# zhouzypaul/fql

Measured on NVIDIA B200. Metric: fql_update_samples_per_sec, higher is better.
Workload: dtype bf16

## Files before the change

fql_b200/csrc/euler_cluster.cu:

```cuda
#include "step.cuh"
#include "tc_prims.cuh"

using namespace tc;

namespace {

constexpr int TILE_M = 128;
constexpr int KB = 64;
constexpr int A_BLK = TILE_M * 128;
constexpr int SUB = 32;
constexpr int A_SUB = TILE_M * SUB * 2;
constexpr int NSUB = 16;
constexpr int MAX_A = 32;
constexpr int NMMA = 4;
#ifndef FQL_EULER_NISS
#define FQL_EULER_NISS 2
#endif
constexpr int NISS = FQL_EULER_NISS;
static_assert(NISS == 1 || NISS == 2 || NISS == 4, "NISS");
constexpr int NEPI = 4;
constexpr int NTHREADS = 32 * (1 + NMMA + NEPI);
constexpr int EPI0 = 32 * (1 + NMMA);

struct EulerArgs {
// ... 112 lines not shown
    const int N = lastl ? a.A : a.H;
    const int col = lastl ? c : (int)j * NCOL + c;
    sBias[i] = (c < NCOL && col < N && !(l == 0 && a.c0)) ? a.params[(int64_t)s * a.arena + a.off_b[l] + col] : 0.f;
  }
  if (threadIdx.x <= a.n_steps) sT[threadIdx.x] = (float)((double)threadIdx.x / (double)a.n_steps);
  tc_fence_before();
  __syncthreads();
  tc_fence_after();
  cluster_sync_all();
  const uint32_t tmem_base = *tmem_slot;
  if (a.t_start && blockIdx.x == 0 && threadIdx.x == 0) a.t_start[0] = gtime();

  if (warp == 0) {
    const bool el = elect_one();
    {
      if (el) mbar_expect_tx(x_full, nkb_x * A_BLK);
      const int xrow = s * a.x_rows_s + a.x_row0 + tile * TILE_M;
      for (int kb = 0; kb < nkb_x; kb++)
        if (el) tma_load_2d(sX + kb * A_BLK, &mapX, x_full, kb * KB, xrow);
      int n_pub = 0;
      int l = 0;
      for (int it = 0; it < total; it++, l = (l + 1 == NL) ? 0 : l + 1) {
        const bool last = (l == NL - 1);
        const int K = (l == 0) ? a.K0 : a.H;
        const int kblocks = (K + KB - 1) / KB;
        if (it > 0) mbar_wait_u(acc_full, (it - 1) & 1);
        if (el) mbar_expect_tx(full_b, kblocks * B_BLK);
        for (int kb = 0; kb < kblocks; kb++) {
          if (!el) continue;
          if constexpr (MODE == MODE_DGRAD) {
// ... 272 lines not shown
  FQL_REQUIRE(smem <= 232448, "euler_cluster_kernel: shared memory %d > 227 KB", smem);
  auto kern = euler_cluster_kernel<NC, AMAX, MODE>;
  static bool attr_set[FQL_MAX_DEVICES] = {};
  const int dev = fql_current_device();
  if (!attr_set[dev]) {
    FQL_CHECK_CUDA(cudaFuncSetAttribute(kern, cudaFuncAttributeMaxDynamicSharedMemorySize, 232448));
    if (NC > 8) FQL_CHECK_CUDA(cudaFuncSetAttribute(kern, cudaFuncAttributeNonPortableClusterSizeAllowed, 1));
    attr_set[dev] = true;
  }
  cudaLaunchConfig_t cfg;
  memset(&cfg, 0, sizeof(cfg));
  cfg.gridDim = dim3(NC * a.tiles * a.S);
  cfg.blockDim = dim3(NTHREADS);
  cfg.dynamicSmemBytes = smem;
  cfg.stream = st;
  cudaLaunchAttribute attr[1];
  attr[0].id = cudaLaunchAttributeClusterDimension;
  attr[0].val.clusterDim.x = NC;
  attr[0].val.clusterDim.y = 1;
  attr[0].val.clusterDim.z = 1;
  cfg.attrs = attr;
  cfg.numAttrs = 1;
  if (query_only) {
    cfg.stream = nullptr;
    if (cudaOccupancyMaxActiveClusters(max_clusters, kern, &cfg) != cudaSuccess) {
      cudaGetLastError();
      *max_clusters = 0;
    }
    return 0;
  }
  const CUtensorMapSwizzle wsw = (NC == 8 || MODE == MODE_DGRAD) ? CU_TENSOR_MAP_SWIZZLE_128B : CU_TENSOR_MAP_SWIZZLE_64B;
  CUtensorMap mapX, mapW, mapWL;
  HMaps mapsH;
  memset(&mapsH, 0, sizeof(mapsH));
  FQL_TRY(make_map_2d(&mapX, f.X0b, a.K0pad, (uint64_t)a.S * f.Mcap0, 64, TILE_M));
  if (MODE == MODE_DGRAD) {
    FQL_TRY(make_map_2d(&mapW, f.shadow, d->hidden, (uint64_t)a.S * a.w_rows_s, 64, NCOL, wsw));
// ... 130 lines not shown
```

fql_b200/csrc/losses.cu:

```cuda
#include "step.cuh"
#include "dp_comm.cuh"

#include <cuda_bf16.h>

namespace {

__device__ __forceinline__ float clip1(float x) { return fminf(fmaxf(x, -1.0f), 1.0f); }

template <int OP>
__device__ float block_reduce(float v, float* sh) {
  const int lane = threadIdx.x & 31, w = threadIdx.x >> 5, nw = (blockDim.x + 31) >> 5;
  v = OP == 0 ? warp_sum(v) : warp_max(v);
  __syncthreads();
  if (lane == 0) sh[w] = v;
  __syncthreads();
  if (w == 0) {
    float x = lane < nw ? sh[lane] : (OP == 0 ? 0.f : -INFINITY);
    x = OP == 0 ? warp_sum(x) : warp_max(x);
    if (lane == 0) sh[0] = x;
  }
  __syncthreads();
  float r = sh[0];
  return r;
}
// ... 196 lines not shown
__global__ void euler_update_kernel(StepShape sh, WsPtrs w, int step) {
  const int A = sh.A, B = sh.B, KF = sh.F + sh.A + 1;
  const int64_t i = (int64_t)blockIdx.x * blockDim.x + threadIdx.x;
  if (i >= (int64_t)sh.S * B * A) return;
  const int c = (int)(i % A);
  const int64_t row = i / A;
  const int s = (int)(row / B), r = (int)(row % B);
  float* xf = w.XF + ((int64_t)s * 2 * B + B + r) * KF;
  const float v = w.F_out[((int64_t)s * 2 * B + B + r) * A + c];
  const float a = xf[sh.F + c] + v / (float)sh.flow_steps;
  xf[sh.F + c] = a;
  if (c == 0) xf[sh.F + A] = (float)((double)(step + 1) / (double)sh.flow_steps);
  if (step == sh.flow_steps - 1) w.target[i] = clip1(a);
}

__global__ void actor_grad_kernel(StepShape sh, FqlHparams hp, WsPtrs w, float* raw, __nv_bfloat16* dapib) {
  __shared__ float red[32];
  const int s = blockIdx.x;
  const int A = sh.A, B = sh.B, KC = sh.F + sh.A;
  const float* api = w.O_out + ((int64_t)s * 3 * B + B) * A;
  const float scale = hp.alpha * 2.0f / ((float)sh.GB * (float)A);
  float sq = 0.f;
  if (dapib) {
    const int P = 64 - A;
    for (int i = blockIdx.y * blockDim.x + threadIdx.x; i < B * P; i += gridDim.y * blockDim.x)
      dapib[((int64_t)s * B + i / P) * 64 + A + i % P] = __float2bfloat16(0.f);
  }
  for (int i = blockIdx.y * blockDim.x + threadIdx.x; i < B * A; i += gridDim.y * blockDim.x) {
    const int r = i / A, c = i % A;
    const float a = api[i];
    const float d = a - w.target[(int64_t)s * B * A + i];
    sq += d * d;
    const float g0 = w.dX0[(((int64_t)s * 2 + 0) * B + r) * KC + sh.F + c];
    const float g1 = w.dX0[(((int64_t)s * 2 + 1) * B + r) * KC + sh.F + c];
    const float inside = (a >= -1.0f && a <= 1.0f) ? 1.0f : 0.0f;
    const float g = scale * d + (g0 + g1) * inside;
    w.dapi[(int64_t)s * B * A + i] = g;
    if (dapib) dapib[((int64_t)s * B + r) * 64 + c] = __float2bfloat16(g);
  }
  sq = block_reduce<0>(sq, red);
  if (threadIdx.x == 0) atomicAdd(&raw[s * FQL_NUM_RAW + RAW_DISTILL_SQ], sq);
}

__global__ void finalize_info_kernel(StepShape sh, FqlHparams hp, const float* raw, int ranks, const float* gstats, float* info,
                                     int with_grad_stats) {
  const int s = blockIdx.x * blockDim.x + threadIdx.x;
  if (s >= sh.S) return;
  fql_finalize_info_seed(sh, hp, raw, ranks, gstats, info, s, with_grad_stats);
}

__global__ void clip_kernel(const float* in, float* out, int64_t n) {
  const int64_t i = (int64_t)blockIdx.x * blockDim.x + threadIdx.x;
  if (i < n) out[i] = clip1(in[i]);
}

__global__ void concat_kernel(const float* x0, int k0, const float* x1, int k1, float c2, int k2, float* out, int64_t rows) {
// ... 46 lines not shown
  FQL_CHECK_LAUNCH();
  return 0;
}
int launch_bc_post(const StepShape& sh, const WsPtrs& w, float* raw, cudaStream_t st) {
  bc_post_kernel<<<dim3(sh.S, loss_ctas(sh)), 1024, 0, st>>>(sh, w, raw);
  FQL_CHECK_LAUNCH();
  return 0;
}
int launch_euler_update(const StepShape& sh, const WsPtrs& w, int step, cudaStream_t st) {
  const int64_t n = (int64_t)sh.S * sh.B * sh.A;
  euler_update_kernel<<<(unsigned)((n + 255) / 256), 256, 0, st>>>(sh, w, step);
  FQL_CHECK_LAUNCH();
  return 0;
}
int launch_actor_grad(const StepShape& sh, const FqlHparams& hp, const WsPtrs& w, float* raw, cudaStream_t st, void* dapib) {
  actor_grad_kernel<<<dim3(sh.S, loss_ctas(sh)), 1024, 0, st>>>(sh, hp, w, raw, reinterpret_cast<__nv_bfloat16*>(dapib));
  FQL_CHECK_LAUNCH();
  return 0;
}
int launch_finalize_info(const StepShape& sh, const FqlHparams& hp, const float* raw, int ranks, const float* gstats, float* info,
                         int with_grad_stats, cudaStream_t st) {
  finalize_info_kernel<<<(sh.S + 63) / 64, 64, 0, st>>>(sh, hp, raw, ranks, gstats, info, with_grad_stats);
  FQL_CHECK_LAUNCH();
  return 0;
}
int launch_clip(const float* in, float* out, int64_t n, cudaStream_t st) {
  if (n == 0) return 0;
  clip_kernel<<<(unsigned)((n + 255) / 256), 256, 0, st>>>(in, out, n);
  FQL_CHECK_LAUNCH();
  return 0;
}
// ... 15 lines not shown
```

fql_b200/csrc/optim.cu:

```cuda
#include "step.cuh"

#include <cuda_bf16.h>

namespace {

constexpr int ADAM_U = 1;
__global__ void __launch_bounds__(256) adam_polyak_stats_kernel(Layout L, FqlHparams hp, float* __restrict__ params,
                                                                float* __restrict__ mu, float* __restrict__ nu,
                                                                const float* __restrict__ grads,
                                                                const float* __restrict__ bc,
                                                                float* __restrict__ partials, __nv_bfloat16* __restrict__ shadow,
                                                                int64_t shadow_seed, int blk0, int blk1, int nblk) {
  const int s = blockIdx.y;
  const int b0 = blk0 + blockIdx.x * ADAM_U;
  const int64_t base = (int64_t)s * L.arena;
  const NetView& tgt = L.net[FQL_NET_TARGET_CRITIC];
  const NetView& cri = L.net[FQL_NET_CRITIC];
  float4 g[ADAM_U], p[ADAM_U], m[ADAM_U], v[ADAM_U], tp[ADAM_U];
  bool act[ADAM_U], pol[ADAM_U];
#pragma unroll
  for (int u = 0; u < ADAM_U; u++) {
    const int64_t off = (int64_t)(b0 + u) * FQL_LEAF_PAD + threadIdx.x * 4;
    act[u] = (b0 + u < blk1) && !(off >= tgt.begin && off < tgt.end);
    pol[u] = act[u] && off >= cri.begin && off < cri.end;
    if (act[u]) {
      g[u] = *reinterpret_cast<const float4*>(grads + base + off);
      p[u] = *reinterpret_cast<const float4*>(params + base + off);
// ... 14 lines not shown
    float pn[4];
    float mx = -INFINITY, mn = INFINITY, sq = 0.f;
#pragma unroll
    for (int i = 0; i < 4; i++) {
      const float gi = gr[i];
      mx = fmaxf(mx, gi);
      mn = fminf(mn, gi);
      sq += gi * gi;
      mr[i] = hp.beta1 * mr[i] + hp.one_minus_beta1 * gi;
      vr[i] = hp.beta2 * vr[i] + hp.one_minus_beta2 * gi * gi;
      const float mhat = mr[i] / bc1;
      const float vhat = vr[i] / bc2;
      pn[i] = pr[i] + (-hp.lr * (mhat / (sqrtf(vhat) + hp.eps)));
    }
    *reinterpret_cast<float4*>(params + base + off) = make_float4(pn[0], pn[1], pn[2], pn[3]);
    if (shadow) {
      __nv_bfloat162 lo = __floats2bfloat162_rn(pn[0], pn[1]), hi = __floats2bfloat162_rn(pn[2], pn[3]);
      *reinterpret_cast<uint2*>(shadow + (int64_t)s * shadow_seed + off) = make_uint2(*reinterpret_cast<uint32_t*>(&lo), *reinterpret_cast<uint32_t*>(&hi));
    }
    *reinterpret_cast<float4*>(mu + base + off) = make_float4(mr[0], mr[1], mr[2], mr[3]);
    *reinterpret_cast<float4*>(nu + base + off) = make_float4(vr[0], vr[1], vr[2], vr[3]);
    if (pol[u]) {
      const int64_t toff = base + off - cri.begin + tgt.begin;
      float4 t4 = tp[u];
      const float omt = hp.one_minus_tau;
      t4.x = pr[0] * hp.tau + t4.x * omt;
      t4.y = pr[1] * hp.tau + t4.y * omt;
      t4.z = pr[2] * hp.tau + t4.z * omt;
      t4.w = pr[3] * hp.tau + t4.w * omt;
      *reinterpret_cast<float4*>(params + toff) = t4;
      if (shadow) {
        __nv_bfloat162 lo = __floats2bfloat162_rn(t4.x, t4.y), hi = __floats2bfloat162_rn(t4.z, t4.w);
        *reinterpret_cast<uint2*>(shadow + (int64_t)s * shadow_seed + (toff - base)) = make_uint2(*reinterpret_cast<uint32_t*>(&lo), *reinterpret_cast<uint32_t*>(&hi));
      }
    }
    mx = warp_max(mx);
    mn = warp_min(mn);
    sq = warp_sum(sq);
    if (lane == 0) { smx[u][w] = mx; smn[u][w] = mn; ssq[u][w] = sq; }
  }
  __syncthreads();
  if (threadIdx.x < ADAM_U && b0 + (int)threadIdx.x < blk1) {
    const int u = threadIdx.x;
    float* part = partials + ((int64_t)s * nblk + b0 + u) * 4;
    const int64_t off = (int64_t)(b0 + u) * FQL_LEAF_PAD;
    const bool a_u = !(off >= tgt.begin && off < tgt.end);
    float a = 0.f, b = 0.f, c = 0.f;
    if (a_u) {
      a = smx[u][0]; b = smn[u][0]; c = ssq[u][0];
#pragma unroll
      for (int i = 1; i < 8; i++) { a = fmaxf(a, smx[u][i]); b = fminf(b, smn[u][i]); c += ssq[u][i]; }
    }
    part[0] = a; part[1] = b; part[2] = c;
  }
}

__global__ void __launch_bounds__(1024) grad_stats_final_kernel(Layout L, const float* __restrict__ partials,
                                                                float* __restrict__ gstats, int32_t* count_inc, FinArgs fin) {
  const int s = blockIdx.x;
  const int nblk = L.leaf_blk[L.n_leaves];
  const float* part = partials + (int64_t)s * nblk * 4;
  const int lane = threadIdx.x & 31, w = threadIdx.x >> 5;
  __shared__ float smx[32], smn[32], snorm[32];
  float wmx = 0.f, wmn = 0.f, wnorm = 0.f;
  for (int leaf = w; leaf < L.n_leaves; leaf += 32) {
    if (L.leaf_net[leaf] == FQL_NET_TARGET_CRITIC) continue;
    float mx = -INFINITY, mn = INFINITY, sq = 0.f;
    const int bend = L.leaf_blk[leaf + 1];
    const float4* p4 = reinterpret_cast<const float4*>(part);
    for (int b0 = L.leaf_blk[leaf] + lane; b0 < bend; b0 += 256) {
      float4 v[8];
#pragma unroll
      for (int u = 0; u < 8; u++) v[u] = (b0 + 32 * u < bend) ? p4[b0 + 32 * u] : make_float4(-INFINITY, INFINITY, 0.f, 0.f);
#pragma unroll
      for (int u = 0; u < 8; u++) {
        mx = fmaxf(mx, v[u].x);
        mn = fminf(mn, v[u].y);
        sq += v[u].z;
      }
    }
    mx = warp_max(mx);
    mn = warp_min(mn);
    sq = warp_sum(sq);
    wmx = fmaxf(wmx, mx);
    wmn = fminf(wmn, mn);
    wnorm += sqrtf(sq);
  }
  if (lane == 0) { smx[w] = wmx; smn[w] = wmn; snorm[w] = wnorm; }
  __syncthreads();
  if (threadIdx.x == 0) {
    float a = smx[0], b = smn[0], c = snorm[0];
    for (int i = 1; i < 32; i++) { a = fmaxf(a, smx[i]); b = fminf(b, smn[i]); c += snorm[i]; }
    gstats[s * 4 + 0] = a;
    gstats[s * 4 + 1] = b;
    gstats[s * 4 + 2] = c;
    if (s == 0 && count_inc) count_inc[0] += 1;
    if (fin.info) fql_finalize_info_seed(fin.sh, fin.hp, fin.raw, fin.ranks, gstats, fin.info, s, 1);
  }
}

__global__ void zero_bc_kernel(float4* p, int64_t n4, const int32_t* __restrict__ count, float beta1, float beta2, float* bc, int* tickets,
                               int n_tickets) {
  const int64_t i = (int64_t)blockIdx.x * blockDim.x + threadIdx.x;
  if (i < n4) p[i] = make_float4(0.f, 0.f, 0.f, 0.f);
  if (tickets && i < n_tickets) tickets[i] = 0;
  if (i == 0 && count) {
    const double t = (double)(count[0] + 1);
    bc[0] = 1.0f - (float)pow((double)beta1, t);
    bc[1] = 1.0f - (float)pow((double)beta2, t);
  }
}

__global__ void target_update_kernel(float* __restrict__ params, __nv_bfloat16* __restrict__ shadow, int64_t arena, int64_t shadow_seed,
// ... 9 lines not shown
  t.w = p.w * tau + t.w * omt;
  *reinterpret_cast<float4*>(params + s * arena + tgt0 + i) = t;
  if (shadow) {
    __nv_bfloat162 lo = __floats2bfloat162_rn(t.x, t.y), hi = __floats2bfloat162_rn(t.z, t.w);
    *reinterpret_cast<uint2*>(shadow + s * shadow_seed + tgt0 + i) = make_uint2(*reinterpret_cast<uint32_t*>(&lo), *reinterpret_cast<uint32_t*>(&hi));
  }
}

__global__ void zero_kernel(float4* p, int64_t n4) {
  const int64_t i = (int64_t)blockIdx.x * blockDim.x + threadIdx.x;
  if (i < n4) p[i] = make_float4(0.f, 0.f, 0.f, 0.f);
}

}

int launch_adam_polyak_stats(const Layout& L, const FqlHparams& hp, int S, float* params, float* mu, float* nu,
                             const float* grads, const float* bc, float* partials, void* shadow, int64_t shadow_seed, cudaStream_t st,
                             int blk0, int blk1) {
  const int nblk = L.leaf_blk[L.n_leaves];
  if (blk1 < 0) blk1 = nblk;
  if (blk1 <= blk0) return 0;
  dim3 grid((blk1 - blk0 + ADAM_U - 1) / ADAM_U, S);
  adam_polyak_stats_kernel<<<grid, 256, 0, st>>>(L, hp, params, mu, nu, grads, bc, partials, reinterpret_cast<__nv_bfloat16*>(shadow), shadow_seed, blk0, blk1,
                                                 nblk);
  FQL_CHECK_LAUNCH();
  return 0;
}

int launch_grad_stats_final(const Layout& L, int S, const float* partials, float* gstats, int32_t* count_inc, cudaStream_t st,
                            const FinArgs* fin) {
  FinArgs f;
  memset(&f, 0, sizeof(f));
  if (fin) f = *fin;
  grad_stats_final_kernel<<<S, 1024, 0, st>>>(L, partials, gstats, count_inc, f);
  FQL_CHECK_LAUNCH();
  return 0;
}

int launch_zero_bc(float* p, int64_t n, const int32_t* count, const FqlHparams& hp, float* bc, cudaStream_t st, int* tickets, int n_tickets) {
  const int64_t n4 = n / 4;
  const int64_t work = n4 > n_tickets ? n4 : n_tickets;
  const unsigned blocks = (unsigned)((work + 255) / 256);
  zero_bc_kernel<<<blocks ? blocks : 1, 256, 0, st>>>(reinterpret_cast<float4*>(p), n4, count, hp.beta1, hp.beta2, bc, tickets, n_tickets);
  FQL_CHECK_LAUNCH();
  return 0;
}

extern "C" int fql_target_update(const FqlDims* d, const FqlHparams* hp, float* params, void* shadow, void* stream) {
  Layout L;
// ... 25 lines not shown
```

fql_b200/csrc/step.cu:

```cuda
#include "step.cuh"
#include "dp_comm.cuh"

#include <cuda_bf16.h>
#include <stdarg.h>

#include <vector>

static thread_local char g_err[1024] = "";
thread_local long long g_fql_launches = 0;
void fql_set_error(const char* fmt, ...) {
  va_list ap;
  va_start(ap, fmt);
  vsnprintf(g_err, sizeof(g_err), fmt, ap);
  va_end(ap);
}

int fql_validate_dims(const FqlDims* d) {
  FQL_REQUIRE(d != nullptr, "dims is NULL");
  FQL_REQUIRE(d->batch >= 1 && d->global_batch >= d->batch, "batch=%d global_batch=%d", d->batch, d->global_batch);
  FQL_REQUIRE(d->obs_dim >= 1 && d->action_dim >= 1, "obs_dim=%d action_dim=%d", d->obs_dim, d->action_dim);
  FQL_REQUIRE(d->hidden >= 1 && d->num_hidden >= 1 && d->num_hidden + 1 <= FQL_MAXL, "hidden=%d num_hidden=%d", d->hidden, d->num_hidden);
  FQL_REQUIRE(d->num_seeds >= 1, "num_seeds=%d", d->num_seeds);
  FQL_REQUIRE(d->flow_steps >= 1, "flow_steps=%d", d->flow_steps);
  FQL_REQUIRE(d->precision == FQL_PRECISION_FP32 || d->precision == FQL_PRECISION_BF16_TC || d->precision == FQL_PRECISION_BF16_ENC,
// ... 115 lines not shown
  carve_pass(c, &w->pF, (int)S, (int)(2 * B), (int)H, NH, (int)A, d->actor_layer_norm, true, simt);
  carve_pass(c, &w->pC, (int)(3 * S * 2), (int)B, (int)H, NH, 1, d->critic_layer_norm, true, simt);
  w->O_out = w->pO.out;
  w->F_out = w->pF.out;
  w->C_out = w->pC.out;
  w->dq = c.take(S * 2 * B);
  w->dqs = c.take(S * 2 * B);
  w->dpred = c.take(S * B * A);
  w->dapi = c.take(S * B * A);
  w->target = c.take(S * B * A);
  w->dX0 = c.take(S * 2 * B * (F + A));
  w->raw_local = c.take(S * FQL_NUM_RAW);
  w->gstats = c.take(S * 4 + 4);
  w->partials = c.take(S * (int64_t)L.leaf_blk[L.n_leaves] * 4);
  w->cpost_part = c.take(2 * S * 64 * 4);
  w->cpost_ticket = reinterpret_cast<int*>(c.take(3 * S + 4));
  if (d->reserved[0] > 0) {
    for (int i = 0; i < 5; i++) w->feat[i] = c.take(S * B * F);
    for (int i = 0; i < 3; i++) w->dfeat[i] = c.take(S * B * F);
    w->dX0F = c.take(S * B * (F + A + 1));
    w->dX0O = c.take(S * B * (F + A));
    w->dX0C = c.take(S * 2 * B * (F + A));
    const bool bwd[5] = {false, true, false, true, true};
    for (int i = 0; i < 5; i++) {
      c.off = (c.off + 255) & ~(size_t)255;
      c.off += enc_carve(d, B, base ? c.base + c.off : nullptr, &w->enc[i], bwd[i]);
    }
  }
  if (d->precision == FQL_PRECISION_BF16_TC) {
    const int64_t kO = round_up64(F + A, 64), kF = round_up64(F + A + 1, 64);
    w->XOb = c.take((S * 3 * B * kO + 1) / 2);
// ... 435 lines not shown
                     float* raw, cudaStream_t S0) {
  const FqlBatch& b = *c.b;
  const FqlDims* d = c.d;
  const int S = sh.S, B = sh.B, H = sh.H, NH = sh.NH;
  const float* P = c.st->params;
  const void* shadow = c.st->shadow;
  typedef __nv_bfloat16 bf16;
  cudaStream_t S1 = ctx->s1, S2 = ctx->s2;
  cudaEvent_t ev_prep = ctx->ev[0], ev_f0 = ctx->ev[1], ev_cpost = ctx->ev[2], ev_euler = ctx->ev[3], ev_s2 = ctx->ev[4], ev_pad = ctx->ev[5];
  const int kO = (int)round_up64(sh.F + sh.A, 64), kF = (int)round_up64(sh.F + sh.A + 1, 64);
  const bool dp_grads = ctx->dp.active && c.do_backward;
  const bool wide = tc_wide_input(d), pix = d->reserved[0] > 0;
  const bool dp_bucketed = dp_grads && !pix;
  bool bc_enc_forked = false;
  FQL_TRY(stamp(ctx, 0, S0));
  FQL_TRY(launch_zero_bc(raw, (int64_t)S * FQL_NUM_RAW, c.do_apply ? c.st->count : nullptr, hp, w.gstats + S * 4, S0, w.cpost_ticket, 3 * S));
  FQL_TRY(encode_observations(c, L, w, S0, ctx));
  FQL_TRY(launch_prep(sh, b, w, S0));
  FQL_TRY(stamp(ctx, 1, S0));
  FQL_CHECK_CUDA(cudaEventRecord(ev_prep, S0));
  FQL_CHECK_CUDA(cudaStreamWaitEvent(S1, ev_prep, 0));

  auto actor = [&](int net, const void* X0b, int K0pad, int rows_cap, int r0, int M, void* const* Hb, void* const* Zb, bool with_z) {
    TcActor t;
    memset(&t, 0, sizeof(t));
    t.d = d; t.L = &L; t.net = net; t.params = P; t.shadow = shadow; t.grads = c.st->grads; t.M = M;
    t.X0b = reinterpret_cast<const bf16*>(X0b) + (int64_t)r0 * K0pad; t.K0pad = K0pad; t.x_ss = (long long)rows_cap * K0pad;
    for (int l = 0; l < NH; l++) {
      t.Hb[l] = reinterpret_cast<bf16*>(Hb[l]) + (int64_t)r0 * H;
      t.Zb[l] = with_z ? reinterpret_cast<bf16*>(Zb[l]) + (int64_t)r0 * H : nullptr;
    }
// ... 200 lines not shown
    FQL_CHECK_CUDA(cudaStreamWaitEvent(S2, ctx->ev[16], 0));
    FQL_TRY(stamp(ctx, 8, S2));
    FQL_TRY(record_early(ctx, S2));
    TcCritic q = cr;
    q.grads = nullptr; q.p = 2; q.X0b = reinterpret_cast<const bf16*>(w.XCb) + (int64_t)2 * S * B * kO;
    q.dOut = w.dqs; q.dOutb = w.C2_dOutb; q.dX0 = w.dX0;
    for (int l = 0; l < NH; l++) { q.dZb[l] = w.C2_dZb[l]; q.dZf[l] = w.C2_dZf[l]; q.dHf[l] = w.C2_dHf[l]; }
    if (big_bwd) FQL_TRY(tc_critic_backward_big(q, w.C_XHb, w.C_DGb, S0));
    else FQL_TRY(tc_critic_backward(q, S0, nullptr, nullptr, &ctx->ev[44]));
    FQL_TRY(stamp(ctx, 6, S0));
    if (dp_bucketed && c.do_apply && ctx->dp_early_adam) {
      const int blk1 = (int)(L.net[FQL_NET_ACTOR_ONESTEP_FLOW].begin / FQL_LEAF_PAD);
      FQL_CHECK_CUDA(cudaEventRecord(ctx->ev[52], S0));
      FQL_CHECK_CUDA(cudaStreamWaitEvent(ctx->sc, ctx->ev[52], 0));
      FQL_CHECK_CUDA(cudaStreamWaitEvent(ctx->sc, ev_euler, 0));
      FQL_TRY(launch_adam_polyak_stats(L, hp, S, c.st->params, c.st->mu, c.st->nu, c.st->grads, w.gstats + S * 4, w.partials, c.st->shadow,
                                       tc_shadow_seed_elems(d, L), ctx->sc, 0, blk1));
      FQL_TRY(stamp(ctx, 9, ctx->sc));
      FQL_CHECK_CUDA(cudaEventRecord(ctx->ev[59], ctx->sc));
      ctx->adam_done_blk = blk1;
    }
  }
  if (bc_enc_forked) FQL_CHECK_CUDA(cudaStreamWaitEvent(S2, ctx->ev[37], 0));
  FQL_CHECK_CUDA(cudaEventRecord(ev_s2, S2));
  FQL_CHECK_CUDA(cudaStreamWaitEvent(S0, ev_euler, 0));
  if (split_metric) FQL_CHECK_CUDA(cudaStreamWaitEvent(S0, ctx->ev[57], 0));
  if (split_cpost) FQL_CHECK_CUDA(cudaStreamWaitEvent(S0, ev_cpost, 0));
  FQL_TRY(launch_actor_grad(sh, hp, w, raw, S0, w.O_dOutb));
  FQL_TRY(stamp(ctx, 7, S0));
  if (c.do_backward) {
    TcActor bo = actor(FQL_NET_ACTOR_ONESTEP_FLOW, w.XOb, kO, 3 * B, B, B, w.O_Hb, w.O_Zb, true);
    int rc = 1;
// ... 62 lines not shown
  FQL_REQUIRE(!(c.d->normalize_q_loss && c.d->global_batch != c.d->batch) || ctx->dp.active,
              "normalize_q_loss with a data-parallel split needs the global mean|q| inside the step (agents/fql.py:74-76): attach a peer-memory "
              "communicator (fql_dp_attach); the fql_step_grads / fql_step_apply split cannot provide it");
  if (ctx->dp.active && c.do_grads) {
    FQL_REQUIRE(c.st->grads == ctx->dp.comm.base[ctx->dp.comm.rank], "data parallel: FqlState.grads must be this rank's symmetric buffer (base[rank])");
    FQL_REQUIRE(c.d->global_batch == (int64_t)c.d->batch * ctx->dp.comm.world && ctx->dp.S == S && !c.raw,
                "data parallel: global_batch must be world x batch (%d x %d), seeds as attached, and the raw accumulators internal", ctx->dp.comm.world, c.d->batch);
  }
  float* raw = c.raw ? c.raw : w.raw_local;
  const float* P = c.st->params;

  if (c.do_grads && !tcm) {
    const FqlBatch& b = *c.b;
    cudaStream_t S1 = ctx->s1, S2 = ctx->s2;
    cudaEvent_t ev_prep = ctx->ev[0], ev_f0 = ctx->ev[1], ev_cpost = ctx->ev[2], ev_euler = ctx->ev[3], ev_s2 = ctx->ev[4];
    FQL_TRY(launch_zero_bc(raw, (int64_t)S * FQL_NUM_RAW, c.do_apply ? c.st->count : nullptr, hp, w.gstats + S * 4, S0, w.cpost_ticket, 3 * S));
    FQL_TRY(encode_observations(c, L, w, S0, ctx));
    FQL_TRY(launch_prep(sh, b, w, S0));
    const bool pix = c.d->reserved[0] > 0;
    FQL_CHECK_CUDA(cudaEventRecord(ev_prep, S0));
    FQL_CHECK_CUDA(cudaStreamWaitEvent(S1, ev_prep, 0));
    FQL_CHECK_CUDA(cudaStreamWaitEvent(S2, ev_prep, 0));

    FwdSpec fF;
    memset(&fF, 0, sizeof(fF));
    fF.P = 1; fF.nv[0] = &L.net[FQL_NET_ACTOR_BC_FLOW]; fF.params = P; fF.arena = L.arena;
    fF.S = S; fF.E = 1; fF.M = 2 * B; fF.H = H; fF.X0 = w.XF; fF.Mcap0 = 2 * B; fF.r0_in = 0;
    fF.buf = &w.pF; fF.r0 = 0; fF.save_z = 1;
    {
      FQL_TRY(mlp_forward(fF, S1));
      FQL_CHECK_CUDA(cudaEventRecord(ev_f0, S1));
// ... 73 lines not shown
      const int64_t t0 = L.net[FQL_NET_TARGET_CRITIC].begin;
      FQL_TRY(dp_reduce_bucket(ctx->dp, 3, 0, t0, raw, S0));
    }
  }

  ctx->adam_done_blk = 0;
  if (c.do_grads && tcm) FQL_TRY(enqueue_grads_tc(ctx, c, L, w, sh, hp, raw, S0));
  int raw_ranks = c.raw_ranks > 1 ? c.raw_ranks : 1;
  const float* raw_fin = raw;
  if (ctx->dp.active && c.do_grads) {
    if (!c.do_backward) FQL_TRY(dp_reduce_bucket(ctx->dp, 2, 0, 0, raw, S0));
    raw_fin = dp_raw_all(ctx->dp);
    raw_ranks = ctx->dp.comm.world;
  }
  if (c.do_apply) {
    if (!c.do_grads) FQL_TRY(launch_zero_bc(nullptr, 0, c.st->count, hp, w.gstats + S * 4, S0));
    const int blk0 = ctx->adam_done_blk;
    const int blk1 = blk0 ? (int)(L.net[FQL_NET_TARGET_CRITIC].begin / FQL_LEAF_PAD) : -1;
    FQL_TRY(launch_adam_polyak_stats(L, hp, S, c.st->params, c.st->mu, c.st->nu, c.st->grads, w.gstats + S * 4, w.partials,
                                     tcm ? c.st->shadow : nullptr, tcm ? tc_shadow_seed_elems(c.d, L) : 0, S0, blk0, blk1));
    FQL_TRY(stamp(ctx, 11, S0));
    if (tcm) {
      FQL_CHECK_CUDA(cudaEventRecord(ctx->ev[50], S0));
      FQL_CHECK_CUDA(cudaStreamWaitEvent(ctx->s1, ctx->ev[50], 0));
      FQL_TRY(tc_refresh_shadow_lastlayer(c.d, L, c.st->params, c.st->shadow, ctx->s1));
      FQL_CHECK_CUDA(cudaEventRecord(ctx->ev[51], ctx->s1));
    }
    FinArgs fin;
    memset(&fin, 0, sizeof(fin));
    fin.sh = sh; fin.hp = hp; fin.raw = raw_fin; fin.ranks = raw_ranks; fin.info = c.info;
    FQL_TRY(launch_grad_stats_final(L, S, w.partials, w.gstats, c.st->count, S0, c.info ? &fin : nullptr));
    if (tcm) FQL_CHECK_CUDA(cudaStreamWaitEvent(S0, ctx->ev[51], 0));
  }
  if (c.info && !c.do_apply) FQL_TRY(launch_finalize_info(sh, hp, raw_fin, raw_ranks, w.gstats, c.info, 0, S0));
  FQL_TRY(stamp(ctx, 12, S0));
  return 0;
}

int run_step_on(FqlContext* ctx, const StepCall& c, cudaStream_t S0) {
  cudaStreamCaptureStatus cap = cudaStreamCaptureStatusNone;
  FQL_CHECK_CUDA(cudaStreamIsCapturing(S0, &cap));
  if (!ctx->use_graph || cap != cudaStreamCaptureStatusNone) {
    const long long before = g_fql_launches;
    const int rc0 = enqueue_step(ctx, c, S0);
    ctx->launches += g_fql_launches - before;
    return rc0;
  }
// ... 343 lines not shown
```

fql_b200/csrc/step.cuh:

```cuda
#pragma once
#include "common.cuh"

#include <cudaTypedefs.h>

enum {
  RAW_CRITIC_SQ = 0, RAW_Q_SUM = 1, RAW_BC_SQ = 2, RAW_DISTILL_SQ = 3, RAW_QPI_SUM = 4, RAW_QPI_ABS = 5, RAW_MSE = 6,
  RAW_Q_MAX = 9, RAW_Q_NEGMIN = 10,
};

struct StepShape {
  int S, B, GB, F, A, H, NH;
  int q_agg_min, normalize_q_loss, flow_steps;
};

struct PassBuf {
  float* Z[FQL_MAXL];
  float* Hh[FQL_MAXL];
  float* mu[FQL_MAXL];
  float* rstd[FQL_MAXL];
  float* out;
  int G, Mcap;
};

struct EncTc {
// ... 7 lines not shown
  uint8_t* arg[3];
  float *flat, *z, *scratch;
  float *dz, *dflat, *da, *db, *dc, *partial;
  int flat_dim;
};

struct WsPtrs {
  float *XO, *XF, *XC, *vel;
  float *O_out, *F_out, *C_out;
  float *dq, *dqs, *dpred, *dapi, *target, *dX0;
  float *raw_local;
  float *gstats;
  float *partials;
  float *cpost_part;
  int *cpost_ticket;
  PassBuf pO, pF, pC;
  float *dC[2], *dCp[2], *dF[2], *dO[2];
  void *XOb, *XFb, *XCb;
  void *O_Hb[FQL_MAXL], *O_Zb[FQL_MAXL], *F_Hb[FQL_MAXL], *F_Zb[FQL_MAXL], *E_Hb[FQL_MAXL];
  void *C_Hb[FQL_MAXL];
  void *C_XHb[FQL_MAXL], *C_DGb[FQL_MAXL];
  void *O_dZb[FQL_MAXL], *F_dZb[FQL_MAXL], *O_dOutb, *F_dOutb;
  float *O_dZf[FQL_MAXL], *F_dZf[FQL_MAXL];
  void *C1_dZb[FQL_MAXL], *C1_dOutb, *C2_dZb[FQL_MAXL], *C2_dOutb;
  float *C1_dZf[FQL_MAXL], *C1_dHf[FQL_MAXL], *C2_dZf[FQL_MAXL], *C2_dHf[FQL_MAXL];
  float *euler_a;
  float *cs_scratch[3];
  float *feat[5];
  float *dfeat[3];
  float *dX0F, *dX0O, *dX0C;
  EncBuf enc[5];
  const float *src[5];
  void *euler_hx;
};

StepShape make_shape(const FqlDims* d);
size_t carve_workspace(const FqlDims* d, const Layout& L, void* base, WsPtrs* w);

int launch_prep(const StepShape& sh, const FqlBatch& b, const WsPtrs& w, cudaStream_t st);
int launch_post_onestep(const StepShape& sh, const FqlBatch& b, const WsPtrs& w, float* raw, cudaStream_t st, int parts = 3);
struct DpLamArgs;
int launch_critic_post(const StepShape& sh, const FqlHparams& hp, const FqlBatch& b, const WsPtrs& w, float* raw, cudaStream_t st, int parts = 3,
                       const DpLamArgs* dpl = nullptr);
int launch_bc_post(const StepShape& sh, const WsPtrs& w, float* raw, cudaStream_t st);
int launch_euler_update(const StepShape& sh, const WsPtrs& w, int step, cudaStream_t st);
int launch_actor_grad(const StepShape& sh, const FqlHparams& hp, const WsPtrs& w, float* raw, cudaStream_t st, void* dapib = nullptr);
int launch_finalize_info(const StepShape& sh, const FqlHparams& hp, const float* raw, int ranks, const float* gstats, float* info,
                         int with_grad_stats, cudaStream_t st);
int launch_clip(const float* in, float* out, int64_t n, cudaStream_t st);
int launch_concat(const float* x0, int k0, const float* x1, int k1, float c2, int k2, float* out, int64_t rows, cudaStream_t st);
int launch_euler_inplace(float* X, const float* v, int F, int A, int64_t rows, int step, int nsteps, float* out, cudaStream_t st);

int launch_adam_polyak_stats(const Layout& L, const FqlHparams& hp, int S, float* params, float* mu, float* nu,
                             const float* grads, const float* bc, float* partials, void* shadow, int64_t shadow_seed, cudaStream_t st,
                             int blk0 = 0, int blk1 = -1);
struct FinArgs {
  StepShape sh;
  FqlHparams hp;
  const float* raw;
  int ranks;
  float* info;
};
int launch_grad_stats_final(const Layout& L, int S, const float* partials, float* gstats, int32_t* count_inc, cudaStream_t st,
                            const FinArgs* fin = nullptr);

#ifdef __CUDACC__
__device__ __forceinline__ void fql_finalize_info_seed(const StepShape& sh, const FqlHparams& hp, const float* raw, int ranks, const float* gstats,
                                                       float* info, int s, int with_grad_stats) {
  float rw[FQL_NUM_RAW];
  for (int i = 0; i < FQL_NUM_RAW; i++) rw[i] = raw[s * FQL_NUM_RAW + i];
  for (int r = 1; r < ranks; r++) {
    const float* o = raw + ((int64_t)r * sh.S + s) * FQL_NUM_RAW;
    for (int i = 0; i < 9; i++) rw[i] += o[i];
    rw[RAW_Q_MAX] = fmaxf(rw[RAW_Q_MAX], o[RAW_Q_MAX]);
    rw[RAW_Q_NEGMIN] = fmaxf(rw[RAW_Q_NEGMIN], o[RAW_Q_NEGMIN]);
  }
  float* o = info + s * FQL_NUM_INFO;
  const float gb = (float)sh.GB, A = (float)sh.A;
  const float critic_loss = rw[RAW_CRITIC_SQ] / (2.0f * gb);
// ... 218 lines not shown
```

Measured before the change: 1.146 million.

## Fuse grad-stats reduction into Adam, add PDL and vectorize actor grad

The separate grad_stats_final kernel and last-layer shadow refresh are removed. The Adam kernel now does a ticket-based last-block reduction per leaf and per seed, and writes the padded bf16 last-layer shadow inline. The actor-grad kernel processes 8 columns per thread with vectorized bf16 stores, finishes its reduction by ticket instead of atomics, and triggers programmatic dependent launch so the DGRAD euler cluster kernel can launch early and wait on griddepcontrol. This cuts kernel launches and cross-stream event syncs, at the cost of more ticket bookkeeping and an extra per-element net scan inside Adam.

```diff
diff --git a/fql_b200/csrc/euler_cluster.cu b/fql_b200/csrc/euler_cluster.cu
--- a/fql_b200/csrc/euler_cluster.cu
+++ b/fql_b200/csrc/euler_cluster.cu
@@ -150,6 +150,7 @@
   if (warp == 0) {
     const bool el = elect_one();
     {
+      if constexpr (MODE == MODE_DGRAD) asm volatile("griddepcontrol.wait;" ::: "memory");
       if (el) mbar_expect_tx(x_full, nkb_x * A_BLK);
       const int xrow = s * a.x_rows_s + a.x_row0 + tile * TILE_M;
       for (int kb = 0; kb < nkb_x; kb++)
@@ -452,13 +453,15 @@
   cfg.blockDim = dim3(NTHREADS);
   cfg.dynamicSmemBytes = smem;
   cfg.stream = st;
-  cudaLaunchAttribute attr[1];
+  cudaLaunchAttribute attr[2];
   attr[0].id = cudaLaunchAttributeClusterDimension;
   attr[0].val.clusterDim.x = NC;
   attr[0].val.clusterDim.y = 1;
   attr[0].val.clusterDim.z = 1;
+  attr[1].id = cudaLaunchAttributeProgrammaticStreamSerialization;
+  attr[1].val.programmaticStreamSerializationAllowed = 1;
   cfg.attrs = attr;
-  cfg.numAttrs = 1;
+  cfg.numAttrs = (MODE == MODE_DGRAD && !query_only && fql_pdl_enabled()) ? 2 : 1;
   if (query_only) {
     cfg.stream = nullptr;
     if (cudaOccupancyMaxActiveClusters(max_clusters, kern, &cfg) != cudaSuccess) {
diff --git a/fql_b200/csrc/losses.cu b/fql_b200/csrc/losses.cu
--- a/fql_b200/csrc/losses.cu
+++ b/fql_b200/csrc/losses.cu
@@ -234,32 +234,58 @@
   if (step == sh.flow_steps - 1) w.target[i] = clip1(a);
 }
 
-__global__ void actor_grad_kernel(StepShape sh, FqlHparams hp, WsPtrs w, float* raw, __nv_bfloat16* dapib) {
+__global__ void __launch_bounds__(256) actor_grad_kernel(StepShape sh, FqlHparams hp, WsPtrs w, float* raw, __nv_bfloat16* dapib) {
   __shared__ float red[32];
+  __shared__ int s_last;
   const int s = blockIdx.x;
   const int A = sh.A, B = sh.B, KC = sh.F + sh.A;
+  const int nch = dapib ? 8 : (A + 7) / 8;
   const float* api = w.O_out + ((int64_t)s * 3 * B + B) * A;
   const float scale = hp.alpha * 2.0f / ((float)sh.GB * (float)A);
   float sq = 0.f;
-  if (dapib) {
-    const int P = 64 - A;
-    for (int i = blockIdx.y * blockDim.x + threadIdx.x; i < B * P; i += gridDim.y * blockDim.x)
-      dapib[((int64_t)s * B + i / P) * 64 + A + i % P] = __float2bfloat16(0.f);
-  }
-  for (int i = blockIdx.y * blockDim.x + threadIdx.x; i < B * A; i += gridDim.y * blockDim.x) {
-    const int r = i / A, c = i % A;
-    const float a = api[i];
-    const float d = a - w.target[(int64_t)s * B * A + i];
-    sq += d * d;
-    const float g0 = w.dX0[(((int64_t)s * 2 + 0) * B + r) * KC + sh.F + c];
-    const float g1 = w.dX0[(((int64_t)s * 2 + 1) * B + r) * KC + sh.F + c];
-    const float inside = (a >= -1.0f && a <= 1.0f) ? 1.0f : 0.0f;
-    const float g = scale * d + (g0 + g1) * inside;
-    w.dapi[(int64_t)s * B * A + i] = g;
-    if (dapib) dapib[((int64_t)s * B + r) * 64 + c] = __float2bfloat16(g);
-  }
+  for (int i = blockIdx.y * blockDim.x + threadIdx.x; i < B * nch; i += gridDim.y * blockDim.x) {
+    const int r = i / nch, c0 = (i % nch) * 8;
+    float gv[8];
+#pragma unroll
+    for (int k = 0; k < 8; k++) {
+      const int c = c0 + k;
+      gv[k] = 0.f;
+      if (c >= A) continue;
+      const int64_t e = (int64_t)r * A + c;
+      const float a = api[e];
+      const float d = a - w.target[(int64_t)s * B * A + e];
+      sq += d * d;
+      const float g0 = w.dX0[(((int64_t)s * 2 + 0) * B + r) * KC + sh.F + c];
+      const float g1 = w.dX0[(((int64_t)s * 2 + 1) * B + r) * KC + sh.F + c];
+      const float inside = (a >= -1.0f && a <= 1.0f) ? 1.0f : 0.0f;
+      const float g = scale * d + (g0 + g1) * inside;
+      w.dapi[(int64_t)s * B * A + e] = g;
+      gv[k] = g;
+    }
+    if (dapib) {
+      uint32_t u[4];
+#pragma unroll
+      for (int k = 0; k < 4; k++) {
+        __nv_bfloat162 v = __floats2bfloat162_rn(gv[2 * k], gv[2 * k + 1]);
+        u[k] = *reinterpret_cast<uint32_t*>(&v);
+      }
+      *reinterpret_cast<uint4*>(dapib + ((int64_t)s * B + r) * 64 + c0) = make_uint4(u[0], u[1], u[2], u[3]);
+    }
+  }
+  asm volatile("griddepcontrol.launch_dependents;" ::: "memory");
   sq = block_reduce<0>(sq, red);
-  if (threadIdx.x == 0) atomicAdd(&raw[s * FQL_NUM_RAW + RAW_DISTILL_SQ], sq);
+  if (threadIdx.x == 0) {
+    w.ag_part[s * FQL_AG_CTAS + blockIdx.y] = sq;
+    __threadfence();
+    s_last = atomicAdd(&w.ag_ticket[s], 1) == (int)gridDim.y - 1;
+  }
+  __syncthreads();
+  if (!s_last) return;
+  __threadfence();
+  float v = 0.f;
+  for (int c = threadIdx.x; c < (int)gridDim.y; c += blockDim.x) v += __ldcg(&w.ag_part[s * FQL_AG_CTAS + c]);
+  v = block_reduce<0>(v, red);
+  if (threadIdx.x == 0) raw[s * FQL_NUM_RAW + RAW_DISTILL_SQ] += v;
 }
 
 __global__ void finalize_info_kernel(StepShape sh, FqlHparams hp, const float* raw, int ranks, const float* gstats, float* info,
@@ -336,7 +362,9 @@
   return 0;
 }
 int launch_actor_grad(const StepShape& sh, const FqlHparams& hp, const WsPtrs& w, float* raw, cudaStream_t st, void* dapib) {
-  actor_grad_kernel<<<dim3(sh.S, loss_ctas(sh)), 1024, 0, st>>>(sh, hp, w, raw, reinterpret_cast<__nv_bfloat16*>(dapib));
+  const int64_t n = (int64_t)sh.B * (dapib ? 8 : (sh.A + 7) / 8);
+  const int ctas = (int)((n + 255) / 256 < FQL_AG_CTAS ? (n + 255) / 256 : FQL_AG_CTAS);
+  actor_grad_kernel<<<dim3(sh.S, ctas), 256, 0, st>>>(sh, hp, w, raw, reinterpret_cast<__nv_bfloat16*>(dapib));
   FQL_CHECK_LAUNCH();
   return 0;
 }
diff --git a/fql_b200/csrc/optim.cu b/fql_b200/csrc/optim.cu
--- a/fql_b200/csrc/optim.cu
+++ b/fql_b200/csrc/optim.cu
@@ -5,12 +5,82 @@
 namespace {
 
 constexpr int ADAM_U = 1;
-__global__ void __launch_bounds__(256) adam_polyak_stats_kernel(Layout L, FqlHparams hp, float* __restrict__ params,
+static_assert(ADAM_U == 1, "the statistics tickets count one block per CTA");
+
+__device__ __forceinline__ int64_t lastlayer_pad_base(const Layout& L, int net) {
+  int64_t base = L.arena;
+  for (int t = 0; t < net; t++) base += (int64_t)L.net[t].ens * L.net[t].hidden * 64;
+  return base;
+}
+
+struct StatsArgs {
+  float* partials;
+  float4* leaf;
+  int* leaf_ticket;
+  int* seed_ticket;
+  float* gstats;
+  int32_t* count_inc;
+  int n_grad_leaves;
+  FinArgs fin;
+};
+
+__device__ __forceinline__ void stats_leaf_done(const Layout& L, const StatsArgs& sa, int s, int leaf, int nblk) {
+  const int lane = threadIdx.x & 31;
+  float mx = -INFINITY, mn = INFINITY, sq = 0.f;
+  const int bend = L.leaf_blk[leaf + 1];
+  const float4* p4 = reinterpret_cast<const float4*>(sa.partials + (int64_t)s * nblk * 4);
+  for (int b0 = L.leaf_blk[leaf] + lane; b0 < bend; b0 += 256) {
+    float4 v[8];
+#pragma unroll
+    for (int u = 0; u < 8; u++) v[u] = (b0 + 32 * u < bend) ? __ldcg(p4 + b0 + 32 * u) : make_float4(-INFINITY, INFINITY, 0.f, 0.f);
+#pragma unroll
+    for (int u = 0; u < 8; u++) {
+      mx = fmaxf(mx, v[u].x);
+      mn = fminf(mn, v[u].y);
+      sq += v[u].z;
+    }
+  }
+  mx = warp_max(mx);
+  mn = warp_min(mn);
+  sq = warp_sum(sq);
+  int last = 0;
+  if (lane == 0) {
+    sa.leaf[(int64_t)s * L.n_leaves + leaf] = make_float4(mx, mn, sqrtf(sq), 0.f);
+    __threadfence();
+    last = atomicAdd(&sa.seed_ticket[s], 1) == sa.n_grad_leaves - 1;
+  }
+  if (!__shfl_sync(0xffffffffu, last, 0)) return;
+  __threadfence();
+  float wmx = 0.f, wmn = 0.f, wnorm = 0.f;
+  for (int l = lane; l < L.n_leaves; l += 32) {
+    if (L.leaf_net[l] == FQL_NET_TARGET_CRITIC) continue;
+    const float4 r = __ldcg(sa.leaf + (int64_t)s * L.n_leaves + l);
+    wmx = fmaxf(wmx, r.x);
+    wmn = fminf(wmn, r.y);
+    wnorm += r.z;
+  }
+  float a = __shfl_sync(0xffffffffu, wmx, 0), b = __shfl_sync(0xffffffffu, wmn, 0), c = __shfl_sync(0xffffffffu, wnorm, 0);
+  for (int i = 1; i < 32; i++) {
+    a = fmaxf(a, __shfl_sync(0xffffffffu, wmx, i));
+    b = fminf(b, __shfl_sync(0xffffffffu, wmn, i));
+    c += __shfl_sync(0xffffffffu, wnorm, i);
+  }
+  if (lane == 0) {
+    sa.gstats[s * 4 + 0] = a;
+    sa.gstats[s * 4 + 1] = b;
+    sa.gstats[s * 4 + 2] = c;
+    if (s == 0 && sa.count_inc) sa.count_inc[0] += 1;
+    const FinArgs& fin = sa.fin;
+    if (fin.info) fql_finalize_info_seed(fin.sh, fin.hp, fin.raw, fin.ranks, sa.gstats, fin.info, s, 1);
+  }
+}
+
+__global__ void __launch_bounds__(256, 5) adam_polyak_stats_kernel(const __grid_constant__ Layout L, FqlHparams hp, float* __restrict__ params,
                                                                 float* __restrict__ mu, float* __restrict__ nu,
                                                                 const float* __restrict__ grads,
-                                                                const float* __restrict__ bc,
-                                                                float* __restrict__ partials, __nv_bfloat16* __restrict__ shadow,
-                                                                int64_t shadow_seed, int blk0, int blk1, int nblk) {
+                                                                const float* __restrict__ bc, __nv_bfloat16* __restrict__ shadow,
+                                                                int64_t shadow_seed, int blk0, int blk1, int nblk,
+                                                                const __grid_constant__ StatsArgs sa) {
   const int s = blockIdx.y;
   const int b0 = blk0 + blockIdx.x * ADAM_U;
   const int64_t base = (int64_t)s * L.arena;
@@ -55,24 +125,43 @@
       pn[i] = pr[i] + (-hp.lr * (mhat / (sqrtf(vhat) + hp.eps)));
     }
     *reinterpret_cast<float4*>(params + base + off) = make_float4(pn[0], pn[1], pn[2], pn[3]);
-    if (shadow) {
-      __nv_bfloat162 lo = __floats2bfloat162_rn(pn[0], pn[1]), hi = __floats2bfloat162_rn(pn[2], pn[3]);
-      *reinterpret_cast<uint2*>(shadow + (int64_t)s * shadow_seed + off) = make_uint2(*reinterpret_cast<uint32_t*>(&lo), *reinterpret_cast<uint32_t*>(&hi));
-    }
     *reinterpret_cast<float4*>(mu + base + off) = make_float4(mr[0], mr[1], mr[2], mr[3]);
     *reinterpret_cast<float4*>(nu + base + off) = make_float4(vr[0], vr[1], vr[2], vr[3]);
+    float4 t4 = make_float4(0.f, 0.f, 0.f, 0.f);
     if (pol[u]) {
       const int64_t toff = base + off - cri.begin + tgt.begin;
-      float4 t4 = tp[u];
+      t4 = tp[u];
       const float omt = hp.one_minus_tau;
       t4.x = pr[0] * hp.tau + t4.x * omt;
       t4.y = pr[1] * hp.tau + t4.y * omt;
       t4.z = pr[2] * hp.tau + t4.z * omt;
       t4.w = pr[3] * hp.tau + t4.w * omt;
       *reinterpret_cast<float4*>(params + toff) = t4;
-      if (shadow) {
-        __nv_bfloat162 lo = __floats2bfloat162_rn(t4.x, t4.y), hi = __floats2bfloat162_rn(t4.z, t4.w);
-        *reinterpret_cast<uint2*>(shadow + (int64_t)s * shadow_seed + (toff - base)) = make_uint2(*reinterpret_cast<uint32_t*>(&lo), *reinterpret_cast<uint32_t*>(&hi));
+    }
+    if (shadow) {
+      __nv_bfloat16* sh = shadow + (int64_t)s * shadow_seed;
+      __nv_bfloat162 lo = __floats2bfloat162_rn(pn[0], pn[1]), hi = __floats2bfloat162_rn(pn[2], pn[3]);
+      *reinterpret_cast<uint2*>(sh + off) = make_uint2(*reinterpret_cast<uint32_t*>(&lo), *reinterpret_cast<uint32_t*>(&hi));
+      if (pol[u]) {
+        lo = __floats2bfloat162_rn(t4.x, t4.y), hi = __floats2bfloat162_rn(t4.z, t4.w);
+        *reinterpret_cast<uint2*>(sh + off - cri.begin + tgt.begin) = make_uint2(*reinterpret_cast<uint32_t*>(&lo), *reinterpret_cast<uint32_t*>(&hi));
+      }
+      const int64_t boff = (int64_t)(b0 + u) * FQL_LEAF_PAD;
+      for (int net = 0; net < FQL_NUM_NETS; net++) {
+        const NetView& nv = L.net[net];
+        const int64_t lw = nv.off_w[nv.n_layers - 1];
+        const int n = nv.ens * nv.hidden * nv.out_dim;
+        if (net == FQL_NET_TARGET_CRITIC || boff < lw || boff >= lw + n) continue;
+        __nv_bfloat16* pad = sh + lastlayer_pad_base(L, net);
+        __nv_bfloat16* tpad = sh + lastlayer_pad_base(L, FQL_NET_TARGET_CRITIC);
+        const float tv[4] = {t4.x, t4.y, t4.z, t4.w};
+        for (int i = 0; i < 4; i++) {
+          const int j = (int)(off - lw) + i;
+          if (j >= n) break;
+          const int dst = (j / nv.out_dim) * 64 + j % nv.out_dim;
+          pad[dst] = __float2bfloat16(pn[i]);
+          if (pol[u]) tpad[dst] = __float2bfloat16(tv[i]);
+        }
       }
     }
     mx = warp_max(mx);
@@ -81,63 +170,29 @@
     if (lane == 0) { smx[u][w] = mx; smn[u][w] = mn; ssq[u][w] = sq; }
   }
   __syncthreads();
-  if (threadIdx.x < ADAM_U && b0 + (int)threadIdx.x < blk1) {
-    const int u = threadIdx.x;
-    float* part = partials + ((int64_t)s * nblk + b0 + u) * 4;
-    const int64_t off = (int64_t)(b0 + u) * FQL_LEAF_PAD;
-    const bool a_u = !(off >= tgt.begin && off < tgt.end);
-    float a = 0.f, b = 0.f, c = 0.f;
-    if (a_u) {
-      a = smx[u][0]; b = smn[u][0]; c = ssq[u][0];
-#pragma unroll
-      for (int i = 1; i < 8; i++) { a = fmaxf(a, smx[u][i]); b = fminf(b, smn[u][i]); c += ssq[u][i]; }
-    }
-    part[0] = a; part[1] = b; part[2] = c;
-  }
-}
-
-__global__ void __launch_bounds__(1024) grad_stats_final_kernel(Layout L, const float* __restrict__ partials,
-                                                                float* __restrict__ gstats, int32_t* count_inc, FinArgs fin) {
-  const int s = blockIdx.x;
-  const int nblk = L.leaf_blk[L.n_leaves];
-  const float* part = partials + (int64_t)s * nblk * 4;
-  const int lane = threadIdx.x & 31, w = threadIdx.x >> 5;
-  __shared__ float smx[32], smn[32], snorm[32];
-  float wmx = 0.f, wmn = 0.f, wnorm = 0.f;
-  for (int leaf = w; leaf < L.n_leaves; leaf += 32) {
-    if (L.leaf_net[leaf] == FQL_NET_TARGET_CRITIC) continue;
-    float mx = -INFINITY, mn = INFINITY, sq = 0.f;
-    const int bend = L.leaf_blk[leaf + 1];
-    const float4* p4 = reinterpret_cast<const float4*>(part);
-    for (int b0 = L.leaf_blk[leaf] + lane; b0 < bend; b0 += 256) {
-      float4 v[8];
-#pragma unroll
-      for (int u = 0; u < 8; u++) v[u] = (b0 + 32 * u < bend) ? p4[b0 + 32 * u] : make_float4(-INFINITY, INFINITY, 0.f, 0.f);
-#pragma unroll
-      for (int u = 0; u < 8; u++) {
-        mx = fmaxf(mx, v[u].x);
-        mn = fminf(mn, v[u].y);
-        sq += v[u].z;
+  __shared__ int s_leaf;
+  if (threadIdx.x == 0) {
+    s_leaf = -1;
+    float* part = sa.partials + ((int64_t)s * nblk + b0) * 4;
+    if (act[0]) {
+      float a = smx[0][0], b = smn[0][0], c = ssq[0][0];
+#pragma unroll
+      for (int i = 1; i < 8; i++) { a = fmaxf(a, smx[0][i]); b = fminf(b, smn[0][i]); c += ssq[0][i]; }
+      part[0] = a; part[1] = b; part[2] = c;
+      __threadfence();
+      int lo = 0, hi = L.n_leaves - 1;
+      while (lo < hi) {
+        const int mid = (lo + hi + 1) >> 1;
+        if (L.leaf_blk[mid] <= b0) lo = mid; else hi = mid - 1;
       }
-    }
-    mx = warp_max(mx);
-    mn = warp_min(mn);
-    sq = warp_sum(sq);
-    wmx = fmaxf(wmx, mx);
-    wmn = fminf(wmn, mn);
-    wnorm += sqrtf(sq);
-  }
-  if (lane == 0) { smx[w] = wmx; smn[w] = wmn; snorm[w] = wnorm; }
+      const int t = atomicAdd(&sa.leaf_ticket[s * L.n_leaves + lo], 1);
+      if (t == L.leaf_blk[lo + 1] - L.leaf_blk[lo] - 1) s_leaf = lo;
+    }
+  }
   __syncthreads();
-  if (threadIdx.x == 0) {
-    float a = smx[0], b = smn[0], c = snorm[0];
-    for (int i = 1; i < 32; i++) { a = fmaxf(a, smx[i]); b = fminf(b, smn[i]); c += snorm[i]; }
-    gstats[s * 4 + 0] = a;
-    gstats[s * 4 + 1] = b;
-    gstats[s * 4 + 2] = c;
-    if (s == 0 && count_inc) count_inc[0] += 1;
-    if (fin.info) fql_finalize_info_seed(fin.sh, fin.hp, fin.raw, fin.ranks, gstats, fin.info, s, 1);
-  }
+  if (s_leaf < 0 || w != 0) return;
+  __threadfence();
+  stats_leaf_done(L, sa, s, s_leaf, nblk);
 }
 
 __global__ void zero_bc_kernel(float4* p, int64_t n4, const int32_t* __restrict__ count, float beta1, float beta2, float* bc, int* tickets,
@@ -177,25 +232,21 @@
 
 }
 
-int launch_adam_polyak_stats(const Layout& L, const FqlHparams& hp, int S, float* params, float* mu, float* nu,
-                             const float* grads, const float* bc, float* partials, void* shadow, int64_t shadow_seed, cudaStream_t st,
+int launch_adam_polyak_stats(const Layout& L, const FqlHparams& hp, int S, float* params, float* mu, float* nu, const float* grads,
+                             const WsPtrs& w, void* shadow, int64_t shadow_seed, int32_t* count_inc, const FinArgs* fin, cudaStream_t st,
                              int blk0, int blk1) {
   const int nblk = L.leaf_blk[L.n_leaves];
   if (blk1 < 0) blk1 = nblk;
   if (blk1 <= blk0) return 0;
+  StatsArgs sa;
+  memset(&sa, 0, sizeof(sa));
+  sa.partials = w.partials; sa.leaf = reinterpret_cast<float4*>(w.leaf_stats); sa.leaf_ticket = w.leaf_ticket; sa.seed_ticket = w.seed_ticket;
+  sa.gstats = w.gstats; sa.count_inc = count_inc;
+  for (int l = 0; l < L.n_leaves; l++) sa.n_grad_leaves += L.leaf_net[l] != FQL_NET_TARGET_CRITIC;
+  if (fin) sa.fin = *fin;
   dim3 grid((blk1 - blk0 + ADAM_U - 1) / ADAM_U, S);
-  adam_polyak_stats_kernel<<<grid, 256, 0, st>>>(L, hp, params, mu, nu, grads, bc, partials, reinterpret_cast<__nv_bfloat16*>(shadow), shadow_seed, blk0, blk1,
-                                                 nblk);
-  FQL_CHECK_LAUNCH();
-  return 0;
-}
-
-int launch_grad_stats_final(const Layout& L, int S, const float* partials, float* gstats, int32_t* count_inc, cudaStream_t st,
-                            const FinArgs* fin) {
-  FinArgs f;
-  memset(&f, 0, sizeof(f));
-  if (fin) f = *fin;
-  grad_stats_final_kernel<<<S, 1024, 0, st>>>(L, partials, gstats, count_inc, f);
+  adam_polyak_stats_kernel<<<grid, 256, 0, st>>>(L, hp, params, mu, nu, grads, w.gstats + S * 4, reinterpret_cast<__nv_bfloat16*>(shadow),
+                                                 shadow_seed, blk0, blk1, nblk, sa);
   FQL_CHECK_LAUNCH();
   return 0;
 }
diff --git a/fql_b200/csrc/step.cu b/fql_b200/csrc/step.cu
--- a/fql_b200/csrc/step.cu
+++ b/fql_b200/csrc/step.cu
@@ -153,7 +153,12 @@
   w->gstats = c.take(S * 4 + 4);
   w->partials = c.take(S * (int64_t)L.leaf_blk[L.n_leaves] * 4);
   w->cpost_part = c.take(2 * S * 64 * 4);
-  w->cpost_ticket = reinterpret_cast<int*>(c.take(3 * S + 4));
+  w->cpost_ticket = reinterpret_cast<int*>(c.take(ws_tickets((int)S, L)));
+  w->ag_ticket = w->cpost_ticket + 3 * S;
+  w->seed_ticket = w->ag_ticket + S;
+  w->leaf_ticket = w->seed_ticket + S;
+  w->ag_part = c.take(S * FQL_AG_CTAS);
+  w->leaf_stats = c.take(S * (int64_t)L.n_leaves * 4);
   if (d->reserved[0] > 0) {
     for (int i = 0; i < 5; i++) w->feat[i] = c.take(S * B * F);
     for (int i = 0; i < 3; i++) w->dfeat[i] = c.take(S * B * F);
@@ -619,7 +624,7 @@
   const bool dp_bucketed = dp_grads && !pix;
   bool bc_enc_forked = false;
   FQL_TRY(stamp(ctx, 0, S0));
-  FQL_TRY(launch_zero_bc(raw, (int64_t)S * FQL_NUM_RAW, c.do_apply ? c.st->count : nullptr, hp, w.gstats + S * 4, S0, w.cpost_ticket, 3 * S));
+  FQL_TRY(launch_zero_bc(raw, (int64_t)S * FQL_NUM_RAW, c.do_apply ? c.st->count : nullptr, hp, w.gstats + S * 4, S0, w.cpost_ticket, ws_tickets(S, L)));
   FQL_TRY(encode_observations(c, L, w, S0, ctx));
   FQL_TRY(launch_prep(sh, b, w, S0));
   FQL_TRY(stamp(ctx, 1, S0));
@@ -850,8 +855,8 @@
       FQL_CHECK_CUDA(cudaEventRecord(ctx->ev[52], S0));
       FQL_CHECK_CUDA(cudaStreamWaitEvent(ctx->sc, ctx->ev[52], 0));
       FQL_CHECK_CUDA(cudaStreamWaitEvent(ctx->sc, ev_euler, 0));
-      FQL_TRY(launch_adam_polyak_stats(L, hp, S, c.st->params, c.st->mu, c.st->nu, c.st->grads, w.gstats + S * 4, w.partials, c.st->shadow,
-                                       tc_shadow_seed_elems(d, L), ctx->sc, 0, blk1));
+      FQL_TRY(launch_adam_polyak_stats(L, hp, S, c.st->params, c.st->mu, c.st->nu, c.st->grads, w, c.st->shadow, tc_shadow_seed_elems(d, L),
+                                       c.st->count, nullptr, ctx->sc, 0, blk1));
       FQL_TRY(stamp(ctx, 9, ctx->sc));
       FQL_CHECK_CUDA(cudaEventRecord(ctx->ev[59], ctx->sc));
       ctx->adam_done_blk = blk1;
@@ -944,7 +949,7 @@
     const FqlBatch& b = *c.b;
     cudaStream_t S1 = ctx->s1, S2 = ctx->s2;
     cudaEvent_t ev_prep = ctx->ev[0], ev_f0 = ctx->ev[1], ev_cpost = ctx->ev[2], ev_euler = ctx->ev[3], ev_s2 = ctx->ev[4];
-    FQL_TRY(launch_zero_bc(raw, (int64_t)S * FQL_NUM_RAW, c.do_apply ? c.st->count : nullptr, hp, w.gstats + S * 4, S0, w.cpost_ticket, 3 * S));
+    FQL_TRY(launch_zero_bc(raw, (int64_t)S * FQL_NUM_RAW, c.do_apply ? c.st->count : nullptr, hp, w.gstats + S * 4, S0, w.cpost_ticket, ws_tickets(S, L)));
     FQL_TRY(encode_observations(c, L, w, S0, ctx));
     FQL_TRY(launch_prep(sh, b, w, S0));
     const bool pix = c.d->reserved[0] > 0;
@@ -1048,23 +1053,15 @@
     raw_ranks = ctx->dp.comm.world;
   }
   if (c.do_apply) {
-    if (!c.do_grads) FQL_TRY(launch_zero_bc(nullptr, 0, c.st->count, hp, w.gstats + S * 4, S0));
+    if (!c.do_grads) FQL_TRY(launch_zero_bc(nullptr, 0, c.st->count, hp, w.gstats + S * 4, S0, w.cpost_ticket, ws_tickets(S, L)));
     const int blk0 = ctx->adam_done_blk;
     const int blk1 = blk0 ? (int)(L.net[FQL_NET_TARGET_CRITIC].begin / FQL_LEAF_PAD) : -1;
-    FQL_TRY(launch_adam_polyak_stats(L, hp, S, c.st->params, c.st->mu, c.st->nu, c.st->grads, w.gstats + S * 4, w.partials,
-                                     tcm ? c.st->shadow : nullptr, tcm ? tc_shadow_seed_elems(c.d, L) : 0, S0, blk0, blk1));
-    FQL_TRY(stamp(ctx, 11, S0));
-    if (tcm) {
-      FQL_CHECK_CUDA(cudaEventRecord(ctx->ev[50], S0));
-      FQL_CHECK_CUDA(cudaStreamWaitEvent(ctx->s1, ctx->ev[50], 0));
-      FQL_TRY(tc_refresh_shadow_lastlayer(c.d, L, c.st->params, c.st->shadow, ctx->s1));
-      FQL_CHECK_CUDA(cudaEventRecord(ctx->ev[51], ctx->s1));
-    }
     FinArgs fin;
     memset(&fin, 0, sizeof(fin));
     fin.sh = sh; fin.hp = hp; fin.raw = raw_fin; fin.ranks = raw_ranks; fin.info = c.info;
-    FQL_TRY(launch_grad_stats_final(L, S, w.partials, w.gstats, c.st->count, S0, c.info ? &fin : nullptr));
-    if (tcm) FQL_CHECK_CUDA(cudaStreamWaitEvent(S0, ctx->ev[51], 0));
+    FQL_TRY(launch_adam_polyak_stats(L, hp, S, c.st->params, c.st->mu, c.st->nu, c.st->grads, w, tcm ? c.st->shadow : nullptr,
+                                     tcm ? tc_shadow_seed_elems(c.d, L) : 0, c.st->count, &fin, S0, blk0, blk1));
+    FQL_TRY(stamp(ctx, 11, S0));
   }
   if (c.info && !c.do_apply) FQL_TRY(launch_finalize_info(sh, hp, raw_fin, raw_ranks, w.gstats, c.info, 0, S0));
   FQL_TRY(stamp(ctx, 12, S0));
diff --git a/fql_b200/csrc/step.cuh b/fql_b200/csrc/step.cuh
--- a/fql_b200/csrc/step.cuh
+++ b/fql_b200/csrc/step.cuh
@@ -45,6 +45,11 @@
   float *partials;
   float *cpost_part;
   int *cpost_ticket;
+  int *ag_ticket;
+  int *seed_ticket;
+  int *leaf_ticket;
+  float *ag_part;
+  float *leaf_stats;
   PassBuf pO, pF, pC;
   float *dC[2], *dCp[2], *dF[2], *dO[2];
   void *XOb, *XFb, *XCb;
@@ -65,6 +70,9 @@
   void *euler_hx;
 };
 
+#define FQL_AG_CTAS 512
+inline int ws_tickets(int S, const Layout& L) { return 5 * S + S * L.n_leaves; }
+
 StepShape make_shape(const FqlDims* d);
 size_t carve_workspace(const FqlDims* d, const Layout& L, void* base, WsPtrs* w);
 
@@ -82,9 +90,6 @@
 int launch_concat(const float* x0, int k0, const float* x1, int k1, float c2, int k2, float* out, int64_t rows, cudaStream_t st);
 int launch_euler_inplace(float* X, const float* v, int F, int A, int64_t rows, int step, int nsteps, float* out, cudaStream_t st);
 
-int launch_adam_polyak_stats(const Layout& L, const FqlHparams& hp, int S, float* params, float* mu, float* nu,
-                             const float* grads, const float* bc, float* partials, void* shadow, int64_t shadow_seed, cudaStream_t st,
-                             int blk0 = 0, int blk1 = -1);
 struct FinArgs {
   StepShape sh;
   FqlHparams hp;
@@ -92,8 +97,9 @@
   int ranks;
   float* info;
 };
-int launch_grad_stats_final(const Layout& L, int S, const float* partials, float* gstats, int32_t* count_inc, cudaStream_t st,
-                            const FinArgs* fin = nullptr);
+int launch_adam_polyak_stats(const Layout& L, const FqlHparams& hp, int S, float* params, float* mu, float* nu, const float* grads,
+                             const WsPtrs& w, void* shadow, int64_t shadow_seed, int32_t* count_inc, const FinArgs* fin, cudaStream_t st,
+                             int blk0 = 0, int blk1 = -1);
 
 #ifdef __CUDACC__
 __device__ __forceinline__ void fql_finalize_info_seed(const StepShape& sh, const FqlHparams& hp, const float* raw, int ranks, const float* gstats,
```

New measurement: 1.135 million (median of 6 runs). No clear change (-1.0%).
